# hasindu2008/slow5tools

Hardware: AMD Instinct MI355X
Metric: blow5_encode_raw_signal_throughput (higher is better)
Workload: dtype int16->u8

## Files before the change

### slow5tools_amd/csrc/deflate2_dev.h

```cpp
#pragma once

namespace s5 {

__device__ __forceinline__ uint32_t alignbit(uint32_t hi, uint32_t lo, uint32_t sh) { return __builtin_amdgcn_alignbit(hi, lo, sh); }
__device__ __forceinline__ uint32_t zbytes(uint32_t x) {
    const uint32_t t = (x & 0x7F7F7F7Fu) + 0x7F7F7F7Fu;
    return ~(t | x | 0x7F7F7F7Fu);
}
__device__ __forceinline__ uint32_t frame_mask(int a0, int first, int len) {
    const int lo = min(4, max(0, first - a0)), hi = min(4, max(0, len - a0));
    const uint32_t mh = hi >= 4 ? 0xFFFFFFFFu : (1u << (8 * hi)) - 1u;
    const uint32_t ml = lo >= 4 ? 0xFFFFFFFFu : (1u << (8 * lo)) - 1u;
    return mh & ~ml & 0x80808080u;
}
__device__ __forceinline__ int top_slot(uint32_t m) { return (31 - __clz((int)m)) >> 3; }

__device__ __forceinline__ void length_symbol(int L, uint32_t &sym, uint32_t &eb, uint32_t &ev) {
    const int l = L - 3;
    eb = 0; ev = 0;
    if (L == 258) sym = 285;
    else if (l < 8) sym = 257 + l;
    else {
        const int nb = 29 - __clz(l);
        sym = 261 + 4 * nb + ((l >> nb) & 3);
// ... 176 lines not shown
                    return C & ((Cp1 & (E | Cm1)) | (Ep & Cm1));
                };
                if (__ballot((member_of(E0, EpA) | member_of(E1, E0)) != 0u) == 0ull) {
                    carryE = (uint32_t)__builtin_amdgcn_readlane((int)E1, 63);
                    const uint32_t bA = alignbit(w0, wp, 16), bB = alignbit(w1, w0, 16);
                    atomicAdd(&wf[bA & 255u], 1u);
                    atomicAdd(&wf[(bA >> 8) & 255u], 1u);
                    atomicAdd(&wf[(bA >> 16) & 255u], 1u);
                    atomicAdd(&wf[bA >> 24], 1u);
                    atomicAdd(&wf[bB & 255u], 1u);
                    atomicAdd(&wf[(bB >> 8) & 255u], 1u);
                    atomicAdd(&wf[(bB >> 16) & 255u], 1u);
                    atomicAdd(&wf[bB >> 24], 1u);
                    const uint32_t wA = (uint32_t)(len - (256 * k + 8 * lane - 2));
                    const uint32_t sA = __builtin_amdgcn_udot4(bA, 0x01010101u, 0u, false), sB = __builtin_amdgcn_udot4(bB, 0x01010101u, 0u, false);
                    a_acc += sA + sB;
                    b_acc = __umul24(wA, sA) + __umul24(wA - 4u, sB) + b_acc;
                    d_acc = __builtin_amdgcn_udot4(bA, 0x03020100u, d_acc, false);
                    d_acc = __builtin_amdgcn_udot4(bB, 0x03020100u, d_acc, false);
                    wc.ok = false;
                    k++;
                    continue;
                }
            }
#endif
            const bool full = k > 0 && 256 * k + 256 <= len;
            const uint32_t wgt = (uint32_t)(len - (256 * k + 4 * lane - 2));
            SlabCls c;
            if (full) c = classify_slab<false>(buf32, k, len, carryE);
            else c = classify_slab<true>(buf32, k, len, carryE);
            const bool anymem = __ballot(c.member != 0u) != 0ull;
            if (full && !anymem) {
                atomicAdd(&wf[c.bytes & 255u], 1u);
                atomicAdd(&wf[(c.bytes >> 8) & 255u], 1u);
                atomicAdd(&wf[(c.bytes >> 16) & 255u], 1u);
                atomicAdd(&wf[c.bytes >> 24], 1u);
                const uint32_t s4 = __builtin_amdgcn_udot4(c.bytes, 0x01010101u, 0u, false);
                a_acc += s4;
                b_acc = __umul24(wgt, s4) + b_acc;
                d_acc = __builtin_amdgcn_udot4(c.bytes, 0x03020100u, d_acc, false);
                wc.ok = false;
                continue;
            }
            {
                uint32_t bytes = c.bytes;
                if (!full) { const uint32_t vb = c.V >> 7; bytes &= (vb << 8) - vb; }
                const uint32_t s4 = __builtin_amdgcn_udot4(bytes, 0x01010101u, 0u, false);
                a_acc += s4;
                b_acc = __umul24(wgt, s4) + b_acc;
                d_acc = __builtin_amdgcn_udot4(bytes, 0x03020100u, d_acc, false);
            }
            const uint32_t lit = c.V & ~c.member;
            if (!anymem) {
#pragma unroll
                for (int q = 0; q < 4; q++)
                    if (lit & (0x80u << (8 * q))) atomicAdd(&wf[(c.bytes >> (8 * q)) & 255u], 1u);
                if (lane == k - k0) segs = SEG_MASK;
                wc.ok = false;
                continue;
            }
            const SlabTail t = slab_tail(buf, k, c, wc);
            uint32_t tsym = 0, teb = 0, tev = 0;
            if (t.ql < 4 && t.rem >= 3) length_symbol((int)t.rem, tsym, teb, tev);
            const uint32_t ntail = t.ql < 4 ? t.nfull + (t.rem >= 3 ? 1u : t.rem) : 0u;
            const uint32_t i1 = (lit >> 7) & 1u, i2 = i1 + ((lit >> 15) & 1u), i3 = i2 + ((lit >> 23) & 1u);
            const uint32_t cnt = i3 + (lit >> 31) + ntail;
            const uint32_t incl = wave_incl_add(cnt);
            const uint32_t total = (uint32_t)__builtin_amdgcn_readlane((int)incl, 63);
            uint32_t st = 0;
            if (lane == 0) {
                st = atomicAdd(&S.lalloc, total);
                if (st < DEFL2_LIST_CAP && st + total > DEFL2_LIST_CAP) {
                    atomicMax(&S.lalloc, (uint32_t)DEFL2_LIST_CAP);
                    st = atomicAdd(&S.lalloc, total);
                }
            }
            st = (uint32_t)__builtin_amdgcn_readfirstlane((int)st);
            const bool listed = st + total <= list_cap && st + total < 65536u;
            uint16_t *tl = st < DEFL2_LIST_CAP ? tla : tlb_top - (st - DEFL2_LIST_CAP) - total - st;
            const uint32_t base = st + incl - cnt;
            const uint32_t idx[4] = {0u, i1, i2, i3};
#pragma unroll
            for (int q = 0; q < 4; q++)
                if (lit & (0x80u << (8 * q))) {
                    const uint32_t b = (c.bytes >> (8 * q)) & 255u;
                    atomicAdd(&wf[b], 1u);
                    if (listed) tl[base + idx[q] + ((uint32_t)q > t.ql ? ntail : 0u)] = (uint16_t)b;
                }
            if (t.ql < 4) {
                uint32_t at = base + (t.ql == 3 ? (lit >> 7) & 1u : 0u);
                if (t.nfull) {
                    atomicAdd(&wf[285], t.nfull);
                    nmatch += t.nfull;
                    if (listed) for (uint32_t i = 0; i < t.nfull; i++) tl[at++] = (uint16_t)285;
                }
                if (t.rem >= 3) {
                    atomicAdd(&wf[tsym], 1u);
                    nmatch += 1;
                    nextra += teb;
                    if (listed) tl[at] = (uint16_t)(tsym | (tev << 9));
                } else if (t.rem) {
                    atomicAdd(&wf[t.runbyte], t.rem);
                    if (listed) for (uint32_t i = 0; i < t.rem; i++) tl[at++] = (uint16_t)t.runbyte;
                }
            }
            if (lane == k - k0) segs = listed ? st | (total << 16) : SEG_REDO;
        }
        const uint32_t a_w = wave_sum(a_acc);
        const uint32_t b_w = wave_sum((b_acc - d_acc) % 65521u);
        const uint32_t mx = wave_sum(nmatch | (nextra << 16));
        if (lane == 0) {
            S.wad[wv] = a_w;
            S.wad[8 + wv] = b_w;
            S.wtot[16 + wv] = mx >> 16;
            S.wtot[24 + wv] = mx & 0xFFFFu;
        }
    }
    __syncthreads();
    if (dbg == 2) { z.bitpos += wfa[tid] + S.wad[tid & 15]; return; }

    const uint32_t la = S.lalloc;
    const uint32_t listb_words = poolb_ok && la > DEFL2_LIST_CAP ? (((la < list_cap ? la : list_cap) - DEFL2_LIST_CAP + 7u) >> 3) << 2 : 0u;
    const bool poolb_used = listb_words != 0u;
    if (wv == 0) {
#ifndef S5_DEFL2_ABSORB
#define S5_DEFL2_ABSORB 2
#endif
        const bool ok = assign_lengths_wave<15, NWV, true, S5_DEFL2_ABSORB>(wfa, NLIT, S.lens, S.blcount, S.bins);
        if (lane == 0) S.dbg = ok ? 0u : 1u;
    } else {
        typedef uint32_t u4a __attribute__((ext_vector_type(4)));
        u4a *o16 = reinterpret_cast<u4a *>(obuf);
        const uint32_t zend = (wf_at - listb_words) / 4;
        for (uint32_t i = (uint32_t)(wv * 64 + lane) - 64u; i < zend; i += TN - 64) o16[i] = u4a{0u, 0u, 0u, 0u};
    }
    __syncthreads();
    if (dbg == 3) { z.bitpos += S.lens[tid]; return; }
    if (tid == 0) {
        if (FUSED) put_bits(obuf, z, 64, 0x9c78u, 16);
        else obuf[0] = z.carry;
    }
    if (wv == 0) {
        if (lane == 0) {
            S.lens[DOFF] = 1; S.lens[DOFF + 1] = 1;
            S.code[DOFF] = 0u | (1u << 16); S.code[DOFF + 1] = 1u | (1u << 16);
        }
        cl_header_wave(S, 2);
    } else if (wv == 1) {
        assign_codes_wave(S.blcount, S.lens, NLIT, S.code);
    } else {
        for (int h = wv - 2; h < NWV; h += NWV - 2) {
            const uint32_t *fh = wfa + h * 288;
            const uint32_t f0 = fh[lane], f1 = fh[64 + lane], f2 = fh[128 + lane], f3 = fh[192 + lane], f4 = lane < NLIT - 256 ? fh[256 + lane] : 0u;
            uint32_t dynb = f0 * S.lens[lane] + f1 * S.lens[64 + lane] + f2 * S.lens[128 + lane] + f3 * S.lens[192 + lane] + f4 * S.lens[256 + lane];
            uint32_t fixb = 8u * (f0 + f1 + f2 + f3 + f4) + (lane >= 16 ? f2 : 0u) + f3 - (lane < 24 ? f4 : 0u);
            dynb = wave_sum(dynb);
            fixb = wave_sum(fixb);
            if (lane == 0) { S.wtot[h] = dynb; S.wtot[8 + h] = fixb; }
            uint32_t *fz = wfa + h * 288;
            fz[lane] = 0u; fz[64 + lane] = 0u; fz[128 + lane] = 0u; fz[192 + lane] = 0u;
            if (lane < NLIT - 256) fz[256 + lane] = 0u;
        }
    }
    __syncthreads();
    if (dbg == 4 || dbg == 41) { z.bitpos += S.wtot[tid & 31] + S.red[6] + S.code[tid]; return; }
    uint32_t my_dyn = 0, my_fix = 0, my_x = 0, my_m = 0;
    if (lane < NWV) { my_dyn = S.wtot[lane]; my_fix = S.wtot[8 + lane]; my_x = S.wtot[16 + lane]; my_m = S.wtot[24 + lane]; }
    auto row8_incl = [](uint32_t v) {
        v += dpp_u32<DPP_ROW_SHR1>(0, v);
        v += dpp_u32<DPP_ROW_SHR2>(0, v);
        if (NWV > 4) v += dpp_u32<DPP_ROW_SHR4>(0, v);
        return v;
    };
    const uint32_t dyn_body_all = (uint32_t)__builtin_amdgcn_readlane((int)row8_incl(my_dyn + my_x + my_m), NWV - 1);
    const uint32_t fix_body_all = (uint32_t)__builtin_amdgcn_readlane((int)row8_incl(my_fix + my_x + 5u * my_m), NWV - 1);
    const uint32_t eob_dyn = S.lens[256];
    const uint32_t hdr_dyn = 17 + 3 * S.hclen + S.red[6];
    const uint32_t dyn_total = hdr_dyn + dyn_body_all + eob_dyn;
    const uint32_t fix_total = 3 + fix_body_all + 7;
    const uint32_t sto_total = 3 + ((0u - (z.bitpos + 3)) & 7) + 32 + 8u * (uint32_t)len;
    if (!FUSED) {
        uint32_t a = 0, b = 0;
#pragma unroll
        for (int w = 0; w < NWV; w++) { a += S.wad[w]; b += S.wad[8 + w]; }
        const uint32_t nb = (uint32_t)(((uint64_t)adB + (uint64_t)len * adA + b) % 65521u);
        adA = (adA + a) % 65521u;
        adB = nb;
    }
    if (sto_total <= dyn_total && sto_total <= fix_total) {
        const uint32_t bytepos = (z.bitpos + 3 + 7) >> 3;
        publish_size(es, (bytepos + 4 + (uint32_t)len) * 8);
        uint8_t *ob8 = reinterpret_cast<uint8_t *>(obuf) + (bytepos - z.flushed * 4);
        if (poolb_used) {
            typedef uint32_t u4a __attribute__((ext_vector_type(4)));
            u4a *l16 = reinterpret_cast<u4a *>(obuf + (wf_at - listb_words));
            for (uint32_t i = tid; i < listb_words / 4; i += TN) l16[i] = u4a{0u, 0u, 0u, 0u};
        }
        __syncthreads();
        if (tid == 0) {
            put_bits(obuf, z, z.bitpos, final ? 1u : 0u, 3);
            put_bits(obuf, z, bytepos * 8, (uint32_t)len | ((~(uint32_t)len) << 16), 32);
        }
        __syncthreads();
        for (int i = tid; i < len; i += TN) ob8[4 + i] = buf[i];
        z.bitpos = (bytepos + 4 + (uint32_t)len) * 8;
        __syncthreads();
        return;
    }
    const bool use_fixed = fix_total < dyn_total || S.dbg != 0;
    const uint32_t dist_bits = use_fixed ? 5u : 1u;
    const uint32_t pos0 = z.bitpos + (use_fixed ? 3u : hdr_dyn);
    const uint32_t my_t = (use_fixed ? my_fix : my_dyn) + my_x + my_m * dist_bits;
    const uint32_t t_incl = row8_incl(my_t);
    const uint32_t total_bits = (uint32_t)__builtin_amdgcn_readlane((int)t_incl, NWV - 1);
    uint32_t wbase = pos0 + (wv ? (uint32_t)__builtin_amdgcn_readlane((int)t_incl, wv - 1) : 0u);
    const uint32_t eob = use_fixed ? fixed_code(256) : S.code[256];
    publish_size(es, pos0 + total_bits + (eob >> 16));
    if (use_fixed) {
        __syncthreads();
        for (int s = tid; s < 288; s += TN) { S.code[s] = fixed_code(s); S.lens[s] = (uint8_t)fixed_len(s); }
    }
    const bool list_ok = !poolb_used || ((pos0 + total_bits + 15u + 31u) >> 5) - z.flushed + 4u <= wf_at - listb_words;
    if (!list_ok) {
        typedef uint32_t u4a __attribute__((ext_vector_type(4)));
        u4a *l16 = reinterpret_cast<u4a *>(obuf + (wf_at - listb_words));
        for (uint32_t i = tid; i < listb_words / 4; i += TN) l16[i] = u4a{0u, 0u, 0u, 0u};
    }
    if (use_fixed || !list_ok) __syncthreads();
    if (wv == 0) {
        if (use_fixed) {
            if (lane == 0) put_bits(obuf, z, z.bitpos, (final ? 1u : 0u) | (1u << 1), 3);
        } else {
            const uint32_t hclen = S.hclen;
            if (lane == 0) put_bits(obuf, z, z.bitpos, (final ? 1u : 0u) | (2u << 1) | ((S.hlit - 257) << 3) | (1u << 8) | ((hclen - 4) << 13), 17);
            if (lane < (int)hclen) {
                const int order[19] = {16, 17, 18, 0, 8, 7, 9, 6, 10, 5, 11, 4, 12, 3, 13, 2, 14, 1, 15};
                put_bits(obuf, z, z.bitpos + 17 + 3 * lane, S.cllens[order[lane]], 3);
            }
            const int ncl = S.ncl;
            uint32_t cv[5], cn[5], sum = 0;
#pragma unroll
            for (int q = 0; q < 5; q++) {
                const int e = 5 * lane + q;
                cv[q] = 0; cn[q] = 0;
                if (e < ncl) {
                    const uint32_t ent = S.clseq[e];
                    const uint32_t sym = ent & 31, cc = S.clcode[sym], cl = cc >> 16;
                    const uint32_t eb = sym == 16 ? 2 : sym == 17 ? 3 : sym == 18 ? 7 : 0;
                    cv[q] = (cc & 0xFFFF) | ((ent >> 5) << cl);
                    cn[q] = cl + eb;
                }
                sum += cn[q];
            }
            uint32_t p = z.bitpos + 17 + 3 * hclen + wave_incl_add(sum) - sum;
#pragma unroll
            for (int q = 0; q < 5; q++) {
                if (cn[q]) put_bits(obuf, z, p, cv[q], cn[q]);
                p += cn[q];
            }
        }
    }
    if (dbg == 5) { z.bitpos += wbase; return; }

    {
        auto or_bits = [&](uint32_t pos, uint64_t v, uint32_t nb) {
            const uint32_t w = (pos >> 5) - z.flushed, sh = pos & 31;
            const uint64_t lo = v << sh;
            atomicOr(&obuf[w], (uint32_t)lo);
            atomicOr(&obuf[w + 1], (uint32_t)(lo >> 32));
            if (sh + nb > 64) atomicOr(&obuf[w + 2], (uint32_t)(v >> (64 - sh)));
        };
        auto lit4 = [&](uint32_t bytes, uint64_t &v, uint32_t &nb) {
            const uint32_t c0 = S.code[bytes & 255u], c1 = S.code[(bytes >> 8) & 255u], c2 = S.code[(bytes >> 16) & 255u], c3 = S.code[bytes >> 24];
            const uint32_t n0 = c0 >> 16, n1 = c1 >> 16, n2 = c2 >> 16, n3 = c3 >> 16;
            const uint32_t lo = (c0 & 0xFFFFu) | ((c1 & 0xFFFFu) << n0), nlo = n0 + n1;
            const uint32_t hi = (c2 & 0xFFFFu) | ((c3 & 0xFFFFu) << n2), nhi = n2 + n3;
            v = (uint64_t)lo | ((uint64_t)hi << nlo);
            nb = nlo + nhi;
        };
        for (int k = k0; k < k1; k++) {
            const uint32_t seg = (uint32_t)__builtin_amdgcn_readlane((int)segs, k - k0);
            if (seg == SEG_FAST && k + 1 < k1 && (uint32_t)__builtin_amdgcn_readlane((int)segs, k + 1 - k0) == SEG_FAST) {
                const int d0 = 64 * k + 2 * lane;
                const uint32_t wp = buf32[d0 - 1], w0 = buf32[d0], w1 = buf32[d0 + 1];
                uint64_t vA, vB;
                uint32_t nA, nB;
                lit4(alignbit(w0, wp, 16), vA, nA);
                lit4(alignbit(w1, w0, 16), vB, nB);
                const uint32_t nb = nA + nB;
                const uint32_t incl = wave_incl_add(nb);
                const uint32_t pos = wbase + incl - nb;
                or_bits(pos, vA, nA);
                or_bits(pos + nA, vB, nB);
                wbase += (uint32_t)__builtin_amdgcn_readlane((int)incl, 63);
                k++;
                continue;
            }
            if (seg == SEG_FAST) {
                const int di = 64 * k + lane;
                uint64_t v;
                uint32_t nb;
                lit4(alignbit(buf32[di], buf32[di - 1], 16), v, nb);
                const uint32_t incl = wave_incl_add(nb);
                or_bits(wbase + incl - nb, v, nb);
                wbase += (uint32_t)__builtin_amdgcn_readlane((int)incl, 63);
                continue;
            }
// ... 111 lines not shown
```

### slow5tools_amd/csrc/deflate_dev.h

```cpp
#pragma once
#include "dev_common.h"

namespace s5 {

constexpr int DEFL_BLK = NT * 64;
constexpr int NLIT = 286;
constexpr int DOFF = 288;

template <int CAP>
struct BuildScratchT {
    alignas(16) uint32_t lf[CAP];
    alignas(16) uint32_t nf[CAP];
    uint16_t npar[CAP];
    uint16_t rsym[CAP];
};
struct SortScratch {
    uint32_t bm[64 * 9];
    uint32_t cnt[64];
    uint32_t ovl[288];
};
struct BuildScratch : BuildScratchT<288> { SortScratch sort; };

struct DeflShared {
    alignas(16) uint32_t freq[320];
// ... 242 lines not shown
            l[q] = lq;
            csum += 1u << (MAXL - lq);
            c[q] = lq > 1 ? 1u << (MAXL - lq) : HUGE_C;
            b[q] = min(63u, (uint32_t)((float)(f[q] << ls) * inv) >> (ls - lq));
        } else { l[q] = 0; c[q] = HUGE_C; b[q] = 0; }
    }
    const uint32_t used_c = wave_sum(csum);
    if (used_c > (1u << MAXL)) return false;
    uint32_t R = (1u << MAXL) - used_c;
    int guard = 0;
    while (R) {
        if (ABSORB > 0 && guard == ABSORB) {
            uint32_t nun = 0;
#pragma unroll
            for (int q = 0; q < 5; q++) nun += (5 * lane + q < n && f[q] == 0u) ? 1u : 0u;
            const uint32_t incl = wave_incl_add(nun);
            if ((uint32_t)__builtin_amdgcn_readlane((int)incl, 63) >= (uint32_t)__popc(R)) {
                uint32_t r = R;
                const uint32_t skip = incl - nun;
#pragma unroll
                for (uint32_t i = 0; i < (uint32_t)MAXL; i++) if (i < skip) r &= r - 1u;
#pragma unroll
                for (int q = 0; q < 5; q++)
                    if (5 * lane + q < n && f[q] == 0u && r) {
                        l[q] = MAXL - (__ffs((int)r) - 1);
                        r &= r - 1u;
                    }
                R = 0;
                break;
            }
        }
        if (++guard > 40) return false;
        bins[lane] = 0;
        wave_sync();
#pragma unroll
        for (int q = 0; q < 5; q++)
            if (c[q] <= R) atomicAdd(&bins[b[q]], c[q]);
        wave_sync();
        const uint32_t hr = bins[63 - lane];
        const uint32_t incl = wave_incl_add(hr);
        const uint64_t fit = __ballot(incl <= R);
        const int nfit = ~fit ? __ffsll((long long)~fit) - 1 : 64;
        const uint32_t whole = nfit ? (uint32_t)__builtin_amdgcn_readlane((int)incl, nfit - 1) : 0u;
        const uint64_t below = nfit < 64 ? (__ballot(hr != 0u) >> nfit) << nfit : 0ull;
        const uint32_t thr = 64u - (uint32_t)nfit;
        const uint32_t pb = below ? 63u - (uint32_t)(__ffsll((long long)below) - 1) : 0xFFFFu;
        const uint32_t Rold = R;
        R -= whole;
        uint32_t mine = 0;
#pragma unroll
        for (int q = 0; q < 5; q++) mine += (c[q] <= Rold && b[q] == pb) ? c[q] : 0u;
        uint32_t run = wave_incl_add(mine) - mine, got = 0;
#pragma unroll
        for (int q = 0; q < 5; q++) {
            bool sel = c[q] <= Rold && b[q] >= thr && b[q] != pb;
            if (c[q] <= Rold && b[q] == pb) { run += c[q]; if (run <= R) { sel = true; got += c[q]; } }
            if (sel) {
                l[q] -= 1;
                c[q] = l[q] > 1 ? c[q] << 1 : HUGE_C;
                b[q] >>= 1;
            }
        }
        R -= wave_sum(got);
    }
#pragma unroll
    for (int q = 0; q < 5; q++) {
        const int s = 5 * lane + q;
        if (s < n) {
            lens[s] = (uint8_t)l[q];
            if (l[q]) atomicAdd(&blcount[l[q]], 1u);
        }
    }
    wave_sync();
    return true;
}

__device__ __forceinline__ void assign_codes_wave(const uint32_t *blcount, const uint8_t *lens, int n, uint32_t *code_out) {
    {
        uint32_t next[16];
        uint32_t c = 0;
        next[0] = 0;
#pragma unroll
        for (int b = 1; b < 16; b++) {
            c = (c + (b > 1 ? (uint32_t)__builtin_amdgcn_readfirstlane((int)blcount[b - 1]) : 0u)) << 1;
            next[b] = c;
        }
        for (int base = 0; base < n; base += 64) {
            const int s = base + lane_id();
            const int l = s < n ? lens[s] : 0;
            uint32_t mine = 0;
#pragma unroll
            for (int b = 1; b < 16; b++) {
                const uint64_t mask = __ballot(l == b);
                if (mask == 0) continue;
                const uint32_t below = __builtin_amdgcn_mbcnt_hi((uint32_t)(mask >> 32), __builtin_amdgcn_mbcnt_lo((uint32_t)mask, 0u));
                if (l == b) mine = next[b] + below;
                next[b] += __popcll(mask);
            }
            if (s < n) code_out[s] = l ? ((__brev(mine) >> (32 - l)) | ((uint32_t)l << 16)) : 0u;
        }
    }
    wave_sync();
}

__device__ __forceinline__ int fixed_len(int s) { return s < 144 ? 8 : s < 256 ? 9 : s < 280 ? 7 : 8; }
__device__ __forceinline__ uint32_t fixed_code(int s) {
    uint32_t c, l;
    if (s < 144) { c = 0x30 + s; l = 8; }
    else if (s < 256) { c = 0x190 + (s - 144); l = 9; }
    else if (s < 280) { c = s - 256; l = 7; }
    else { c = 0xC0 + (s - 280); l = 8; }
    return (__brev(c) >> (32 - l)) | (l << 16);
}

__device__ __forceinline__ void cl_header_wave(DeflShared &S, int hdist) {
    const int lane = lane_id();
    if (lane < 20) S.clfreq[lane] = 0;
    int hl = lane < 29 && S.lens[257 + lane] ? 258 + lane : 257;
    const int hlit = __builtin_amdgcn_readlane(wave_incl_max(hl), 63), n = hlit + hdist;
    if (lane == 0) S.hlit = (uint32_t)hlit;
    wave_sync();
    {
        constexpr int PP = 5;
        const int p0 = PP * lane;
        int v[PP];
        int prevv = -1;
        if (p0 - 1 >= 0 && p0 - 1 < n) prevv = p0 - 1 < hlit ? S.lens[p0 - 1] : S.lens[DOFF + p0 - 1 - hlit];
        uint32_t bk = 0;
#pragma unroll
        for (int q = 0; q < PP; q++) {
            const int p = p0 + q;
            v[q] = p < n ? (p < hlit ? S.lens[p] : S.lens[DOFF + p - hlit]) : -2 - q;
            if (p < n && v[q] != (q == 0 ? prevv : v[q - 1])) bk |= 1u << q;
        }
        const int local_last = bk ? p0 + 31 - __clz(bk) : -1;
        const int local_first = bk ? p0 + __ffs(bk) - 1 : n;
        int lastb = wave_incl_max(local_last);
        lastb = __shfl_up(lastb, 1);
        if (lane == 0) lastb = -1;
        int nextb = wave_suffix_incl_min(local_first);
        nextb = __shfl_down(nextb, 1);
        if (lane == 63) nextb = n;
        uint32_t ent[PP], nent = 0;
#pragma unroll
        for (int q = 0; q < PP; q++) {
            const int p = p0 + q;
            ent[q] = 0xFFFFFFFFu;
            if (p >= n) continue;
            const uint32_t lo = bk & ((2u << q) - 1), hi = bk >> (q + 1);
            const int s = lo ? p0 + 31 - __clz(lo) : lastb;
            const int e = hi ? p + __ffs(hi) : nextb;
            const int R = e - s, rel = p - s;
            if (v[q] == 0) {
                const int c = rel / 138, off = rel - c * 138, Lc = min(138, R - c * 138);
                if (Lc >= 11) { if (off == 0) ent[q] = 18u | ((uint32_t)(Lc - 11) << 5); }
                else if (Lc >= 3) { if (off == 0) ent[q] = 17u | ((uint32_t)(Lc - 3) << 5); }
                else ent[q] = 0;
            } else if (rel == 0) {
                ent[q] = (uint32_t)v[q];
            } else {
                const int mm = rel - 1, c = mm / 6, off = mm - c * 6, Lc = min(6, R - 1 - c * 6);
                if (Lc >= 3) { if (off == 0) ent[q] = 16u | ((uint32_t)(Lc - 3) << 5); }
                else ent[q] = (uint32_t)v[q];
            }
            nent += ent[q] != 0xFFFFFFFFu;
        }
        const uint32_t incl = wave_incl_add(nent);
        uint32_t at = incl - nent;
#pragma unroll
        for (int q = 0; q < PP; q++)
            if (ent[q] != 0xFFFFFFFFu) {
                S.clseq[at++] = (uint16_t)ent[q];
                atomicAdd(&S.clfreq[ent[q] & 31], 1u);
            }
        if (lane == 63) S.ncl = incl;
    }
    wave_sync();
    {
        static constexpr uint32_t CLA[19] = {0x30001, 0x7002f, 0x7006f, 0x7001f, 0x7005f, 0x50003, 0x50013, 0x5000b, 0x5001b, 0x50007,
                                             0x30005, 0x20000, 0x20002, 0x7003f, 0x00000, 0x00000, 0x50017, 0x6000f, 0x7007f};
        static constexpr uint32_t CLB[19] = {0x30002, 0x60017, 0x7002f, 0x7006f, 0x60037, 0x5000b, 0x40005, 0x5001b, 0x50007, 0x4000d,
                                             0x30006, 0x30001, 0x20000, 0x7001f, 0x7005f, 0x7003f, 0x40003, 0x6000f, 0x7007f};
        const uint32_t ca = lane < 19 ? CLA[lane] : 0u, cb = lane < 19 ? CLB[lane] : 0u;
        const uint32_t f = lane < 19 ? S.clfreq[lane] : 0u;
        const uint32_t eb = lane == 16 ? 2u : lane == 17 ? 3u : lane == 18 ? 7u : 0u;
        const uint32_t costA = wave_sum(f * ((ca >> 16) + eb) + ((f && !(ca >> 16)) ? (1u << 24) : 0u));
        const uint32_t costB = wave_sum(f * ((cb >> 16) + eb));
        const bool useA = costA <= costB;
        if (lane < 19) { const uint32_t c = useA ? ca : cb; S.clcode[lane] = c; S.cllens[lane] = (uint8_t)(c >> 16); }
        if (lane == 0) { S.red[6] = useA ? costA : costB; S.hclen = useA ? 18u : 19u; }
    }
}

template <int TN = NT>
__device__ __forceinline__ void flush_words(uint32_t *obuf, uint32_t *out32, ZOut &z, bool final_all, uint32_t n_words = 0xFFFFFFFFu) {
    const int tid = threadIdx.x;
    const uint32_t full = final_all ? (z.bitpos + 31) >> 5 : z.bitpos >> 5;
    const uint32_t n = n_words != 0xFFFFFFFFu ? n_words : full - z.flushed;
    {
        typedef uint32_t u4u __attribute__((ext_vector_type(4), aligned(4)));
        typedef uint32_t u4a __attribute__((ext_vector_type(4)));
        const u4a *s16 = reinterpret_cast<const u4a *>(obuf);
        const uint32_t nv = n >> 2;
        for (uint32_t j = tid; j < nv; j += TN) {
            const uint32_t w = z.flushed + 4u * j;
            const u4a v = s16[j];
            if (w >= 2) *reinterpret_cast<u4u *>(out32 + w) = v;
            else { out32[w + 2] = v.z; out32[w + 3] = v.w; }
        }
        for (uint32_t i = 4u * nv + tid; i < n; i += TN) {
            const uint32_t w = z.flushed + i;
            if (w >= 2) out32[w] = obuf[i];
        }
    }
    if (final_all) return;
    __syncthreads();
    const uint32_t partial = obuf[n];
    __syncthreads();
    for (uint32_t i = tid; i <= n; i += TN) obuf[i] = i == 0 ? partial : 0u;
    __syncthreads();
    z.flushed = full;
}

}
#include "deflate2_dev.h"
namespace s5 {

template <typename M>
__device__ __forceinline__ uint32_t zlib_frame_fused(DeflShared &S, uint32_t *obuf, uint32_t obuf_words, const uint8_t *pay,
                                                     uint32_t plen, ZOut &z, uint32_t dbg = 0, EarlySize es = EarlySize{nullptr, 0}, uint32_t gen_hint = 0,
                                                     bool prepared = false) {
    const int tid = threadIdx.x;
    z.bitpos = 80;
    z.flushed = 0;
    uint32_t adA = 1, adB = 0;
    deflate_block2<1, NT>(S, obuf, obuf_words, pay, (int)plen, true, z, adA, adB, dbg, es, gen_hint, prepared);
    if (dbg) return 16;
    z.bitpos = (z.bitpos + 7) & ~7u;
    if (tid == 0 && plen) {
        uint32_t a = 0, b = 0;
        for (int w = 0; w < NW; w++) { a += S.wad[w]; b += S.wad[8 + w]; }
        adB = (uint32_t)(((uint64_t)plen + b) % 65521u);
        adA = (1u + a) % 65521u;
    }
    if (tid == 0) put_bits(obuf, z, z.bitpos, __builtin_bswap32((adB << 16) | adA), 32);
    z.bitpos += 32;
    __syncthreads();
    return z.bitpos >> 3;
}

template <typename M>
__device__ __forceinline__ uint32_t zlib_compress_fused(DeflShared &S, uint32_t *obuf, uint32_t obuf_words,
                                                        const uint8_t *pay, uint32_t plen, uint8_t *out, uint32_t dbg = 0, uint32_t gen_hint = 0, bool prepared = false) {
    ZOut z;
    const uint32_t total = zlib_frame_fused<M>(S, obuf, obuf_words, pay, plen, z, dbg, EarlySize{nullptr, 0}, gen_hint, prepared);
    if (dbg) {
        if (threadIdx.x == 0) *reinterpret_cast<uint32_t *>(out) = z.bitpos;
        if (dbg == 41 && threadIdx.x < 20) reinterpret_cast<uint32_t *>(out)[4 + threadIdx.x] = threadIdx.x < 19 ? S.clfreq[threadIdx.x] : S.red[6];
        return 16;
    }
    flush_words(obuf, reinterpret_cast<uint32_t *>(out), z, true);
    if (threadIdx.x == 0) *reinterpret_cast<uint64_t *>(out) = (uint64_t)(total - 8);
    return total;
}

constexpr uint64_t LB_MASK = (1ull << 62) - 1;
__device__ __forceinline__ uint64_t wave_sum64(uint64_t v) {
#pragma unroll
    for (int d = 32; d >= 1; d >>= 1) v += __shfl_xor(v, d);
    return v;
}
template <int E = 1>
__device__ __forceinline__ uint64_t lookback_offset(unsigned long long *st, uint32_t r, uint64_t mysize, uint32_t *err, bool published) {
    const int lane = lane_id();
    if (!published && lane == 0) __hip_atomic_store(&st[r], (1ull << 62) | mysize, __ATOMIC_RELAXED, __HIP_MEMORY_SCOPE_AGENT);
    uint64_t acc = 0;
    long long base = (long long)r - 1;
    uint32_t spins = 0;
    for (;;) {
        uint64_t v[E];
#pragma unroll
        for (int e = 0; e < E; e++) {
            const long long idx = base - 64 * e - lane;
            v[e] = idx >= 0 ? __hip_atomic_load(&st[idx], __ATOMIC_RELAXED, __HIP_MEMORY_SCOPE_AGENT) : (2ull << 62);
        }
        int outcome = 0;
#pragma unroll
        for (int e = 0; e < E; e++) {
            if (outcome) continue;
            const uint32_t f = (uint32_t)(v[e] >> 62);
            const uint64_t m0 = __ballot(f == 0), m2 = __ballot(f == 2);
            const int first0 = m0 ? __ffsll((long long)m0) - 1 : 64;
            const int first2 = m2 ? __ffsll((long long)m2) - 1 : 64;
            if (first2 < first0) {
                acc += lane <= first2 ? (v[e] & LB_MASK) : 0ull;
                outcome = 1;
            } else {
                acc += lane < first0 ? (v[e] & LB_MASK) : 0ull;
                if (first0 < 64) { base -= 64 * e + first0; outcome = 2; }
            }
        }
        if (outcome == 1) break;
        if (outcome == 0) { base -= 64 * E; continue; }
        if (++spins > (1u << 22)) { if (lane == 0) *err = 1; break; }
        __builtin_amdgcn_s_sleep(2);
    }
    const uint64_t excl = wave_sum64(acc);
    if (lane == 0) __hip_atomic_store(&st[r], (2ull << 62) | (excl + mysize), __ATOMIC_RELAXED, __HIP_MEMORY_SCOPE_AGENT);
    return excl;
}
__device__ __forceinline__ void copy_record_out(const uint32_t *obuf, uint32_t total, uint8_t *dst) {
    const int tid = threadIdx.x;
    typedef uint32_t u4u __attribute__((ext_vector_type(4), aligned(1)));
    typedef uint32_t u4a __attribute__((ext_vector_type(4)));
// ... 10 lines not shown
```

### slow5tools_amd/csrc/kernels.hip

```cpp
#include <hip/hip_runtime.h>
#include <limits.h>
#include <stdint.h>
#include <stdio.h>
#include <stdlib.h>
#include <string.h>

#include <atomic>
#include <mutex>
#include <type_traits>
#include <vector>

#include "../../include/slow5gpu.h"
#include "deflate_dev.h"
#include "lz_dev.h"
#include "inflate_dev.h"
#include "inflate_simt_dev.h"
#include "inflate_par_dev.h"
#include "zstd_dev.h"
#include "zstd_enc_dev.h"
#include "svb_dev.h"
#include "exzd_dev.h"
#include "order_dev.h"
#include "enc_plan.h"

using namespace s5;

extern "C" void s5gpu_set_error(const char *fmt, ...);
int s5host_set_option(const char *key, long value);
extern uint32_t s5host_generation;
static_assert(s5plan::BLK == (uint32_t)DEFL_BLK && s5plan::SIG_SVB_ZD == S5GPU_SIG_SVB_ZD && s5plan::SIG_EX_ZD == S5GPU_SIG_EX_ZD, "enc_plan.h restates these");

#define HIP_TRY(x)                                                                                   \
    do {                                                                                             \
        hipError_t e_ = (x);                                                                         \
        if (e_ != hipSuccess) {                                                                      \
            s5gpu_set_error("%s failed: %s (%s:%d)", #x, hipGetErrorString(e_), __FILE__, __LINE__); \
            return S5GPU_ERR_HIP;                                                                    \
        }                                                                                            \
    } while (0)

extern __shared__ __attribute__((aligned(16))) uint8_t smem[];

constexpr uint32_t S_BYTES = (sizeof(DeflShared) + 15u) & ~15u;
constexpr uint32_t BZ_BYTES = (sizeof(BuildScratch) + 15u) & ~15u;
constexpr uint32_t B_BYTES = NW * 288u * 4u + 64u;
constexpr uint32_t OVF = 0xFFFFFFFFu;

struct EncParams {
    s5gpu_encode_args_t a;
    uint32_t obuf_words;
    uint32_t pay_cap;
    uint32_t dbg;
    uint32_t zseq;
    uint32_t tier = 0;
};

static uint32_t g_fused_tier2 = 0;
static uint32_t g_zstd_sequences = 1;

__device__ __forceinline__ uint32_t payload_bound_dev(const s5gpu_read_desc_t &d, int sig_method) {
    const uint32_t n = d.n_samples;
    const uint32_t sig = sig_method == S5GPU_SIG_SVB_ZD ? 4 + ((n + 3) >> 2) + 3 * n
                       : sig_method == S5GPU_SIG_EX_ZD ? 24 + 2 * (((n + 3) >> 2) + 4 * n) + n : 2 * n;
    return d.hdr_len + 8 + sig + d.aux_len;
}

template <bool EXZD = false>
__device__ __forceinline__ uint32_t build_payload(const s5gpu_encode_args_t &a, const s5gpu_read_desc_t &d,
                                                  uint8_t *pay, uint32_t cap, uint32_t *ws, uint32_t *red = nullptr) {
    const int tid = threadIdx.x;
    const uint32_t n = d.n_samples;
    if constexpr (EXZD) {
        const uint32_t fixed_x = d.hdr_len + 8 + d.aux_len;
        if (fixed_x + 16 > cap) return OVF;
        const uint8_t *hdr = a.hdr + d.hdr_off;
        for (uint32_t i = tid; i < d.hdr_len; i += NT) pay[i] = hdr[i];
        uint8_t *lenp = pay + d.hdr_len;
        const uint32_t blen = exzd_encode_wg(a.sig + d.sig_off, n, lenp + 8, ws, red, cap - fixed_x);
        if (blen == EXZD_ERR) return OVF;
        if (tid < 8) lenp[tid] = tid < 4 ? (uint8_t)(blen >> (8 * tid)) : 0;
        if (d.aux_len) {
            const uint8_t *aux = a.aux + d.aux_off;
            uint8_t *ap = lenp + 8 + blen;
            for (uint32_t i = tid; i < d.aux_len; i += NT) ap[i] = aux[i];
        }
        return d.hdr_len + 8 + blen + d.aux_len;
    } else {
    const bool svb = a.sig_method == S5GPU_SIG_SVB_ZD;
    const uint32_t nk = (n + 3) >> 2;
    const uint32_t fixed = d.hdr_len + 8 + (svb ? 4 + nk : 0) + d.aux_len;
    if (fixed > cap || (svb ? n : 2 * n) > cap - fixed) return OVF;
    const uint8_t *hdr = a.hdr + d.hdr_off;
    for (uint32_t i = tid; i < d.hdr_len; i += NT) pay[i] = hdr[i];
    uint8_t *lenp = pay + d.hdr_len;
    uint8_t *sigp = lenp + 8;
    const int16_t *sig = a.sig + d.sig_off;
    uint64_t L;
    uint32_t sig_bytes;
    if (svb) {
        uint8_t *keys = sigp + 4;
        uint8_t *data = keys + nk;
        uint32_t total = 0;
        const uint32_t room = cap - fixed;
        for (uint32_t t0 = 0; t0 < n; t0 += SVB_TILE) {
            const uint32_t t = svb_encode_tile(sig, n, t0, keys + (t0 >> 2), data + total, ws, room - total, true);
            if (t > room - total) return OVF;
            total += t;
        }
        L = 4ull + nk + total;
        sig_bytes = (uint32_t)L;
        if (tid < 4) sigp[tid] = (uint8_t)(n >> (8 * tid));
    } else {
        L = n;
        sig_bytes = 2 * n;
        const uint8_t *src = reinterpret_cast<const uint8_t *>(sig);
        for (uint32_t i = tid; i < sig_bytes; i += NT) sigp[i] = src[i];
    }
    if (tid < 8) lenp[tid] = (uint8_t)(L >> (8 * tid));
    if (d.aux_len) {
        const uint8_t *aux = a.aux + d.aux_off;
        uint8_t *ap = sigp + sig_bytes;
        for (uint32_t i = tid; i < d.aux_len; i += NT) ap[i] = aux[i];
    }
    return d.hdr_len + 8 + sig_bytes + d.aux_len;
    }
}

__device__ __forceinline__ uint32_t build_payload_hbm(const s5gpu_encode_args_t &a, const s5gpu_read_desc_t &d, uint8_t *pay,
                                                      uint32_t *ws, uint32_t *tile_keys, uint32_t *tile_data) {
    const int tid = threadIdx.x;
    const uint32_t n = d.n_samples;
    if (a.sig_method == S5GPU_SIG_EX_ZD) return build_payload<true>(a, d, pay, OVF - 1, ws, tile_keys );
    if (a.sig_method != S5GPU_SIG_SVB_ZD) return build_payload(a, d, pay, OVF - 1, ws);
    const uint32_t nk = (n + 3) >> 2;
    const uint8_t *hdr = a.hdr + d.hdr_off;
    for (uint32_t i = tid; i < d.hdr_len; i += NT) pay[i] = hdr[i];
    uint8_t *lenp = pay + d.hdr_len;
    uint8_t *sigp = lenp + 8;
    const int16_t *sig = a.sig + d.sig_off;
    uint8_t *keys = sigp + 4;
    uint8_t *data = keys + nk;
    uint32_t total = 0;
    for (uint32_t t0 = 0; t0 < n; t0 += SVB_TILE) {
        const uint32_t t = svb_encode_tile(sig, n, t0, reinterpret_cast<uint8_t *>(tile_keys), reinterpret_cast<uint8_t *>(tile_data), ws, OVF - 1);
        __syncthreads();
        const uint32_t tk = (min(n - t0, (uint32_t)SVB_TILE) + 3) >> 2;
        copy_record_out(tile_keys, tk, keys + (t0 >> 2));
        copy_record_out(tile_data, t, data + total);
        total += t;
        __syncthreads();
    }
    const uint64_t L = 4ull + nk + total;
    if (tid < 4) sigp[tid] = (uint8_t)(n >> (8 * tid));
    if (tid < 8) lenp[tid] = (uint8_t)(L >> (8 * tid));
    if (d.aux_len) {
        const uint8_t *aux = a.aux + d.aux_off;
        uint8_t *ap = sigp + (uint32_t)L;
        for (uint32_t i = tid; i < d.aux_len; i += NT) ap[i] = aux[i];
    }
    return d.hdr_len + 8 + (uint32_t)L + d.aux_len;
}

__device__ __forceinline__ uint32_t run_heavy_front(const s5gpu_encode_args_t &a, const s5gpu_read_desc_t &d) {
    return a.sig_method == S5GPU_SIG_SVB_ZD ? d.hdr_len + 12u + ((d.n_samples + 3u) >> 2) : 0u;
}

#ifndef S5_FUSED_HINT
#define S5_FUSED_HINT(a, d) run_heavy_front(a, d)
#endif

#ifndef S5_FUSED_WG_PER_CU
#define S5_FUSED_WG_PER_CU 8
#endif
template <typename M, bool EXZD = false, int WPS = S5_FUSED_WG_PER_CU>
__global__ __launch_bounds__(NT, WPS) void k_encode_fused(EncParams p) {
    const uint32_t r = blockIdx.x;
    if (p.tier == 2 && p.a.out_len[r] != 0) return;
    DeflShared &S = *reinterpret_cast<DeflShared *>(smem);
    uint32_t *obuf = reinterpret_cast<uint32_t *>(smem + S_BYTES);
    uint8_t *pay = smem + S_BYTES + 4u * p.obuf_words;
    const s5gpu_read_desc_t d = p.a.desc[r];
    deflate2_prepare<NT>(S, obuf, p.obuf_words);
    const uint32_t plen = build_payload<EXZD>(p.a, d, pay, p.pay_cap, S.ws, S.red);
    if (plen == OVF) {
        if (threadIdx.x == 0 && p.tier != 1) {
            const uint32_t at = atomicAdd(&p.a.ovf[0], 1u);
            p.a.ovf[1 + at] = r;
        }
        return;
    }
    __syncthreads();
    if (p.dbg == 1) {
        if (threadIdx.x == 0) p.a.out_len[r] = plen + pay[plen - 1];
        return;
    }
    uint8_t *out = p.a.slots + d.out_off;
    const uint32_t total = zlib_compress_fused<M>(S, obuf, p.obuf_words, pay, plen, out, p.dbg, S5_FUSED_HINT(p.a, d), true);
    if (threadIdx.x == 0) p.a.out_len[r] = total;
}

#ifndef S5_LB_E
#define S5_LB_E 1
#endif
struct StreamParams {
    unsigned long long *state;
    uint32_t *ctl;
    uint8_t *stream;
    uint64_t *rec_off;
};
template <typename M, bool EXZD = false>
__global__ __launch_bounds__(NT, S5_FUSED_WG_PER_CU) void k_encode_stream(EncParams p, StreamParams sp) {
    __shared__ uint32_t s_r;
    __shared__ uint64_t s_off;
    DeflShared &S = *reinterpret_cast<DeflShared *>(smem);
    uint32_t *obuf = reinterpret_cast<uint32_t *>(smem + S_BYTES);
    uint8_t *pay = smem + S_BYTES + 4u * p.obuf_words;
#ifdef S5_ES_NOTICKET
    const uint32_t r = blockIdx.x;
#else
    if (threadIdx.x == 0) s_r = atomicAdd(&sp.ctl[1], 1u);
    __syncthreads();
    const uint32_t r = s_r;
#endif
    const s5gpu_read_desc_t d = p.a.desc[r];
    deflate2_prepare<NT>(S, obuf, p.obuf_words);
    const uint32_t plen = build_payload<EXZD>(p.a, d, pay, p.pay_cap, S.ws, S.red);
    uint32_t total = 0;
    if (plen == OVF) {
        if (threadIdx.x == 0) atomicAdd(&sp.ctl[0], 1u);
    } else {
        __syncthreads();
        ZOut z;
        total = zlib_frame_fused<M>(S, obuf, p.obuf_words, pay, plen, z, 0, EarlySize{sp.state, r}, S5_FUSED_HINT(p.a, d), true);
        if (threadIdx.x == 0) { obuf[0] = total - 8; obuf[1] = 0; }
    }
    if (wave_id() == 0) {
        const uint64_t off = lookback_offset<S5_LB_E>(sp.state, r, total, &sp.ctl[2], plen != OVF);
        if (lane_id() == 0) {
            s_off = off;
            sp.rec_off[r] = off;
            if (r == p.a.n_reads - 1) sp.rec_off[p.a.n_reads] = off + total;
            p.a.out_len[r] = total;
        }
    }
    __syncthreads();
    if (total) copy_record_out(obuf, total, sp.stream + s_off);
}

__device__ __forceinline__ uint32_t park_offset(const s5gpu_read_desc_t &d, int sig_method) {
    return (d.slot_cap - payload_bound_dev(d, sig_method)) & ~15u;
}

#ifndef S5_PACK_WG
#define S5_PACK_WG 8
#endif
__global__ __launch_bounds__(NT, S5_PACK_WG) void k_pack(EncParams p, int mode, const uint32_t *ord) {
    __shared__ uint32_t ws[16];
    __shared__ __attribute__((aligned(16))) uint32_t tile_keys[SVB_TILE / 16 + 4];
// ... 1865 lines not shown
```

### slow5tools_amd/csrc/svb_dev.h

```cpp
#pragma once
#include "dev_common.h"

namespace s5 {

constexpr int SVB_TILE = NT * 16;

struct SvbTileLane {
    uint32_t z[16];
    uint32_t key, nbytes;
    int valid;
};
#ifndef S5_SVB_PACKED
#define S5_SVB_PACKED 1
#endif
__device__ __forceinline__ void svb_tile_classify(const int16_t *__restrict__ sig, uint32_t n, uint32_t t0, SvbTileLane &T) {
    const int tid = threadIdx.x;
    const uint32_t i0 = t0 + 16u * tid;
    const int valid = i0 >= n ? 0 : (int)min(16u, n - i0);
#if S5_SVB_PACKED
    {
        typedef unsigned short us2 __attribute__((ext_vector_type(2)));
        typedef short ss2 __attribute__((ext_vector_type(2)));
        auto U = [](uint32_t v) { return __builtin_bit_cast(us2, v); };
        auto W = [](us2 v) { return __builtin_bit_cast(uint32_t, v); };
        uint32_t w[8] = {0u, 0u, 0u, 0u, 0u, 0u, 0u, 0u}, pw = 0u;
        bool ok = valid == 0;
        if (valid == 16) {
            const uint4 a = *reinterpret_cast<const uint4 *>(sig + i0);
            const uint4 b = *reinterpret_cast<const uint4 *>(sig + i0 + 8);
            w[0] = a.x; w[1] = a.y; w[2] = a.z; w[3] = a.w; w[4] = b.x; w[5] = b.y; w[6] = b.z; w[7] = b.w;
            if (i0 > 0) pw = *reinterpret_cast<const uint32_t *>(sig + i0 - 2);
            uint32_t rng = W(U(pw) + us2{0x4000, 0x4000});
#pragma unroll
            for (int j = 0; j < 8; j++) rng |= W(U(w[j]) + us2{0x4000, 0x4000});
            ok = (rng & 0x80008000u) == 0u;
        }
        if (__ballot(!ok) == 0ull) {
            uint32_t A = 0, B = 0;
#pragma unroll
            for (int j = 0; j < 8; j++) {
                const uint32_t xp = __builtin_amdgcn_alignbit(w[j], j ? w[j - 1] : pw, 16);
                const ss2 d = __builtin_bit_cast(ss2, w[j]) - __builtin_bit_cast(ss2, xp);
                const us2 z = __builtin_bit_cast(us2, d) << us2{1, 1} ^ __builtin_bit_cast(us2, d >> ss2{15, 15});
                const us2 c = __builtin_elementwise_min(z >> us2{8, 8}, us2{1, 1});
                T.z[2 * j] = (uint32_t)z.x;
                T.z[2 * j + 1] = (uint32_t)z.y;
                if (j < 4) A |= W(c) << (4 * j); else B |= W(c) << (4 * (j - 4));
            }
            const uint32_t key = ((A | (A >> 14)) & 0xFFFFu) | ((B | (B >> 14)) << 16);
            T.key = key;
            T.nbytes = valid == 16 ? 16u + (uint32_t)__popc(key) : 0u;
            T.valid = valid;
            return;
        }
    }
#endif
    int x[16];
    int prev = 0;
    if (valid == 16) {
        const int4 a = *reinterpret_cast<const int4 *>(sig + i0);
        const int4 b = *reinterpret_cast<const int4 *>(sig + i0 + 8);
        const int w[8] = {a.x, a.y, a.z, a.w, b.x, b.y, b.z, b.w};
#pragma unroll
        for (int q = 0; q < 8; q++) {
            x[2 * q] = (int)(short)(w[q] & 0xFFFF);
            x[2 * q + 1] = w[q] >> 16;
        }
    } else {
#pragma unroll
        for (int q = 0; q < 16; q++) x[q] = q < valid ? (int)sig[i0 + q] : 0;
    }
    if (valid > 0 && i0 > 0) prev = sig[i0 - 1];
    uint32_t key = 0, nbytes = 0;
    const bool full = valid == 16;
#pragma unroll
    for (int q = 0; q < 16; q++) {
        const int d = x[q] - prev;
        prev = x[q];
        T.z[q] = ((uint32_t)d << 1) ^ (uint32_t)(d >> 31);
    }
    if (full) {
#pragma unroll
        for (int q = 0; q < 16; q++) {
            const uint32_t code = (T.z[q] > 0xFFu ? 1u : 0u) + (T.z[q] >> 16);
            key |= code << (2 * q);
            nbytes += code;
        }
        nbytes += 16;
    } else {
#pragma unroll
        for (int q = 0; q < 16; q++) {
            const uint32_t code = (T.z[q] > 0xFFu) + (T.z[q] > 0xFFFFu);
            if (q < valid) {
                key |= code << (2 * q);
                nbytes += code + 1;
            }
        }
    }
    T.key = key;
    T.nbytes = nbytes;
    T.valid = valid;
}
__device__ __forceinline__ void svb_tile_write(const SvbTileLane &T, uint8_t *keys, uint8_t *dp) {
    const int tid = threadIdx.x;
    if (T.valid == 16) {
#pragma unroll
        for (int q = 0; q < 16; q++) {
            *dp++ = (uint8_t)T.z[q];
            if (T.z[q] > 0xFFu) {
                *dp++ = (uint8_t)(T.z[q] >> 8);
                if (T.z[q] > 0xFFFFu) *dp++ = (uint8_t)(T.z[q] >> 16);
            }
        }
    } else {
#pragma unroll
        for (int q = 0; q < 16; q++) {
            if (q < T.valid) {
                *dp++ = (uint8_t)T.z[q];
                if (T.z[q] > 0xFFu) *dp++ = (uint8_t)(T.z[q] >> 8);
                if (T.z[q] > 0xFFFFu) *dp++ = (uint8_t)(T.z[q] >> 16);
            }
        }
    }
    const int nk = (T.valid + 3) >> 2;
#pragma unroll
    for (int q = 0; q < 4; q++)
        if (q < nk) keys[4 * tid + q] = (uint8_t)(T.key >> (8 * q));
}
__device__ __forceinline__ uint32_t svb_encode_tile(const int16_t *__restrict__ sig, uint32_t n, uint32_t t0,
                                                    uint8_t *keys, uint8_t *data, uint32_t *ws, uint32_t room, bool ws_fresh = false) {
    SvbTileLane T;
    svb_tile_classify(sig, n, t0, T);
    if (t0 == 0 && !ws_fresh) __syncthreads();
    uint32_t total;
    const uint32_t off = block_excl_add_alt(T.nbytes, ws, total, t0 / (uint32_t)SVB_TILE);
    if (total > room) return total;
    svb_tile_write(T, keys, data + off);
    return total;
}

__device__ __forceinline__ uint32_t svb_key_bytes(uint32_t n) { return (uint32_t)(((uint64_t)n + 3u) >> 2); }
__device__ __forceinline__ bool svb_count_fits(uint32_t n, uint64_t L) { return 4ull + svb_key_bytes(n) + n <= L; }

constexpr uint32_t SVB_STAGE = 4u * SVB_TILE + 16u;
__device__ __forceinline__ uint32_t svb_decode_tile(const uint8_t *keys, const uint8_t *data, const uint8_t *data_end,
                                                    uint32_t n, uint32_t t0, int16_t *__restrict__ out, int &carry,
                                                    int &err, uint32_t *ws, uint8_t *stage) {
    const int tid = threadIdx.x;
    const uint32_t i0 = t0 + 16u * tid;
    const int valid = i0 >= n ? 0 : (int)min(16u, n - i0);
    const int nk = (valid + 3) >> 2;
    uint32_t key = 0;
#pragma unroll
    for (int q = 0; q < 4; q++)
        if (q < nk) key |= (uint32_t)keys[4 * tid + q] << (8 * q);
    uint32_t nbytes = 0;
#pragma unroll
    for (int q = 0; q < 16; q++)
        if (q < valid) nbytes += ((key >> (2 * q)) & 3) + 1;
    uint32_t total;
    const uint32_t off = block_excl_add(nbytes, ws, total);
    {
        const uint32_t have = data < data_end ? (uint32_t)min((uint64_t)total, (uint64_t)(data_end - data)) : 0u;
        typedef uint32_t v4u __attribute__((ext_vector_type(4), aligned(1)));
        typedef uint32_t v4a __attribute__((ext_vector_type(4)));
        for (uint32_t k = 16u * tid; k < have; k += 16u * NT) {
            if (k + 16 <= have) *reinterpret_cast<v4a *>(stage + k) = *reinterpret_cast<const v4u *>(data + k);
            else for (uint32_t j = k; j < have; j++) stage[j] = data[j];
        }
        __syncthreads();
    }
    const uint8_t *dp = stage + off;
    const bool ok = !(valid > 0 && data + off + nbytes > data_end);
    if (!ok) { err = 1; }
    int d[16];
    int sum = 0;
#pragma unroll
    for (int q = 0; q < 16; q++) {
        d[q] = 0;
        if (q < valid && ok) {
            const uint32_t code = (key >> (2 * q)) & 3;
            uint32_t zz = dp[0];
            if (code > 0) zz |= (uint32_t)dp[1] << 8;
            if (code > 1) zz |= (uint32_t)dp[2] << 16;
            if (code > 2) zz |= (uint32_t)dp[3] << 24;
            dp += code + 1;
            d[q] = (int)(zz >> 1) ^ -(int)(zz & 1);
        }
        sum += d[q];
    }
    uint32_t tsum;
    const uint32_t before = block_excl_add((uint32_t)sum, ws, tsum);
    int acc = carry + (int)before;
    if (valid == 16) {
        uint32_t w[8];
#pragma unroll
        for (int q = 0; q < 8; q++) {
            acc += d[2 * q];
            const uint32_t lo = (uint32_t)acc & 0xFFFFu;
            acc += d[2 * q + 1];
            w[q] = lo | ((uint32_t)acc << 16);
        }
        uint4 *o = reinterpret_cast<uint4 *>(out + i0);
        o[0] = make_uint4(w[0], w[1], w[2], w[3]);
        o[1] = make_uint4(w[4], w[5], w[6], w[7]);
    } else {
#pragma unroll
        for (int q = 0; q < 16; q++)
            if (q < valid) { acc += d[q]; out[i0 + q] = (int16_t)acc; }
    }
    carry += (int)tsum;
    return total;
}

constexpr uint32_t SVB_WTILE = 64u * 16u;
constexpr uint32_t SVB_WSTAGE = 4u * SVB_WTILE + 16u;
template <bool STAGED = true>
__device__ __forceinline__ uint32_t svb_decode_tile_wave(const uint8_t *keys, const uint8_t *data, const uint8_t *data_end, uint32_t n, uint32_t t0,
                                                         int16_t *__restrict__ out, int &carry, int &err, uint8_t *stage) {
    const int lane = lane_id();
    const uint32_t i0 = t0 + 16u * (uint32_t)lane;
    const int valid = i0 >= n ? 0 : (int)min(16u, n - i0);
    const int nk = (valid + 3) >> 2;
    uint32_t key = 0;
    if (valid == 16) {
        typedef uint32_t u1 __attribute__((aligned(1)));
        key = *reinterpret_cast<const u1 *>(keys + 4 * lane);
    } else {
#pragma unroll
        for (int q = 0; q < 4; q++)
            if (q < nk) key |= (uint32_t)keys[4 * lane + q] << (8 * q);
    }
    uint32_t nbytes;
    {
        const uint32_t km = valid >= 16 ? key : key & ((1u << (2 * valid)) - 1u);
        uint32_t c = (km & 0x33333333u) + ((km >> 2) & 0x33333333u);
        c = (c + (c >> 4)) & 0x0F0F0F0Fu;
        nbytes = (uint32_t)valid + ((c * 0x01010101u) >> 24);
    }
    const uint32_t incl = wave_incl_add(nbytes);
    const uint32_t off = incl - nbytes;
    const uint32_t total = (uint32_t)__builtin_amdgcn_readlane((int)incl, 63);
    if (STAGED) {
        const uint32_t have = data < data_end ? (uint32_t)min((uint64_t)total, (uint64_t)(data_end - data)) : 0u;
        typedef uint32_t v4u __attribute__((ext_vector_type(4), aligned(1)));
        typedef uint32_t v4a __attribute__((ext_vector_type(4)));
        for (uint32_t k = 16u * (uint32_t)lane; k < have; k += 16u * 64u) {
            if (k + 16 <= have) *reinterpret_cast<v4a *>(stage + k) = *reinterpret_cast<const v4u *>(data + k);
            else for (uint32_t j = k; j < have; j++) stage[j] = data[j];
        }
        wave_sync();
    }
    const uint8_t *dp = (STAGED ? stage : data) + off;
    const bool ok = !(valid > 0 && data + off + nbytes > data_end);
    if (!ok) err = 1;
    int dlt[16];
    int sum = 0;
#pragma unroll
    for (int q = 0; q < 16; q++) {
        dlt[q] = 0;
        if (q < valid && ok) {
            const uint32_t code = (key >> (2 * q)) & 3;
            uint32_t zz = dp[0];
            if (code > 0) zz |= (uint32_t)dp[1] << 8;
            if (code > 1) zz |= (uint32_t)dp[2] << 16;
            if (code > 2) zz |= (uint32_t)dp[3] << 24;
            dp += code + 1;
            dlt[q] = (int)(zz >> 1) ^ -(int)(zz & 1);
        }
        sum += dlt[q];
    }
    const uint32_t incl2 = wave_incl_add((uint32_t)sum);
    int acc = carry + (int)(incl2 - (uint32_t)sum);
    if (valid == 16) {
        uint32_t w[8];
#pragma unroll
        for (int q = 0; q < 8; q++) {
            acc += dlt[2 * q];
            const uint32_t lo = (uint32_t)acc & 0xFFFFu;
            acc += dlt[2 * q + 1];
            w[q] = lo | ((uint32_t)acc << 16);
        }
        uint4 *o = reinterpret_cast<uint4 *>(out + i0);
        o[0] = make_uint4(w[0], w[1], w[2], w[3]);
        o[1] = make_uint4(w[4], w[5], w[6], w[7]);
    } else {
#pragma unroll
        for (int q = 0; q < 16; q++)
            if (q < valid) { acc += dlt[q]; out[i0 + q] = (int16_t)acc; }
    }
// ... 7 lines not shown
```

Before: 687.1.

## Pack SVB zigzag values as 16-bit pairs and write bytes with carry-chained cursors

```diff
diff --git a/slow5tools_amd/csrc/deflate2_dev.h b/slow5tools_amd/csrc/deflate2_dev.h
--- a/slow5tools_amd/csrc/deflate2_dev.h
+++ b/slow5tools_amd/csrc/deflate2_dev.h
@@ -352,7 +352,7 @@
         for (int h = wv - 2; h < NWV; h += NWV - 2) {
             const uint32_t *fh = wfa + h * 288;
             const uint32_t f0 = fh[lane], f1 = fh[64 + lane], f2 = fh[128 + lane], f3 = fh[192 + lane], f4 = lane < NLIT - 256 ? fh[256 + lane] : 0u;
-            uint32_t dynb = f0 * S.lens[lane] + f1 * S.lens[64 + lane] + f2 * S.lens[128 + lane] + f3 * S.lens[192 + lane] + f4 * S.lens[256 + lane];
+            uint32_t dynb = __umul24(f0, S.lens[lane]) + __umul24(f1, S.lens[64 + lane]) + __umul24(f2, S.lens[128 + lane]) + __umul24(f3, S.lens[192 + lane]) + __umul24(f4, S.lens[256 + lane]);
             uint32_t fixb = 8u * (f0 + f1 + f2 + f3 + f4) + (lane >= 16 ? f2 : 0u) + f3 - (lane < 24 ? f4 : 0u);
             dynb = wave_sum(dynb);
             fixb = wave_sum(fixb);
diff --git a/slow5tools_amd/csrc/deflate_dev.h b/slow5tools_amd/csrc/deflate_dev.h
--- a/slow5tools_amd/csrc/deflate_dev.h
+++ b/slow5tools_amd/csrc/deflate_dev.h
@@ -418,14 +418,14 @@
             const int e = hi ? p + __ffs(hi) : nextb;
             const int R = e - s, rel = p - s;
             if (v[q] == 0) {
-                const int c = rel / 138, off = rel - c * 138, Lc = min(138, R - c * 138);
+                const int c = (rel >= 138) + (rel >= 276), off = rel - c * 138, Lc = min(138, R - c * 138);
                 if (Lc >= 11) { if (off == 0) ent[q] = 18u | ((uint32_t)(Lc - 11) << 5); }
                 else if (Lc >= 3) { if (off == 0) ent[q] = 17u | ((uint32_t)(Lc - 3) << 5); }
                 else ent[q] = 0;
             } else if (rel == 0) {
                 ent[q] = (uint32_t)v[q];
             } else {
-                const int mm = rel - 1, c = mm / 6, off = mm - c * 6, Lc = min(6, R - 1 - c * 6);
+                const int mm = rel - 1, c = (int)(__umul24((uint32_t)mm, 171u) >> 10), off = mm - c * 6, Lc = min(6, R - 1 - c * 6);
                 if (Lc >= 3) { if (off == 0) ent[q] = 16u | ((uint32_t)(Lc - 3) << 5); }
                 else ent[q] = (uint32_t)v[q];
             }
diff --git a/slow5tools_amd/csrc/kernels.hip b/slow5tools_amd/csrc/kernels.hip
--- a/slow5tools_amd/csrc/kernels.hip
+++ b/slow5tools_amd/csrc/kernels.hip
@@ -103,7 +103,7 @@
         uint32_t total = 0;
         const uint32_t room = cap - fixed;
         for (uint32_t t0 = 0; t0 < n; t0 += SVB_TILE) {
-            const uint32_t t = svb_encode_tile(sig, n, t0, keys + (t0 >> 2), data + total, ws, room - total, true);
+            const uint32_t t = svb_encode_tile<true>(sig, n, t0, keys + (t0 >> 2), data + total, ws, room - total, true);
             if (t > room - total) return OVF;
             total += t;
         }
diff --git a/slow5tools_amd/csrc/svb_dev.h b/slow5tools_amd/csrc/svb_dev.h
--- a/slow5tools_amd/csrc/svb_dev.h
+++ b/slow5tools_amd/csrc/svb_dev.h
@@ -9,10 +9,17 @@
     uint32_t z[16];
     uint32_t key, nbytes;
     int valid;
+    bool pairs;
 };
 #ifndef S5_SVB_PACKED
 #define S5_SVB_PACKED 1
 #endif
+__device__ __forceinline__ uint32_t svb_pair_codes(uint32_t z) {
+    uint32_t c;
+    asm("v_pk_lshrrev_b16 %0, 8, %1 op_sel_hi:[0,1]\n\tv_pk_min_u16 %0, %0, 1 op_sel_hi:[1,0]" : "=v"(c) : "v"(z));
+    return c;
+}
+template <bool PAIRS = false>
 __device__ __forceinline__ void svb_tile_classify(const int16_t *__restrict__ sig, uint32_t n, uint32_t t0, SvbTileLane &T) {
     const int tid = threadIdx.x;
     const uint32_t i0 = t0 + 16u * tid;
@@ -42,15 +49,22 @@
                 const uint32_t xp = __builtin_amdgcn_alignbit(w[j], j ? w[j - 1] : pw, 16);
                 const ss2 d = __builtin_bit_cast(ss2, w[j]) - __builtin_bit_cast(ss2, xp);
                 const us2 z = __builtin_bit_cast(us2, d) << us2{1, 1} ^ __builtin_bit_cast(us2, d >> ss2{15, 15});
-                const us2 c = __builtin_elementwise_min(z >> us2{8, 8}, us2{1, 1});
-                T.z[2 * j] = (uint32_t)z.x;
-                T.z[2 * j + 1] = (uint32_t)z.y;
-                if (j < 4) A |= W(c) << (4 * j); else B |= W(c) << (4 * (j - 4));
+                uint32_t c;
+                if constexpr (PAIRS) {
+                    c = svb_pair_codes(W(z));
+                    T.z[j] = W(z);
+                } else {
+                    c = W(__builtin_elementwise_min(z >> us2{8, 8}, us2{1, 1}));
+                    T.z[2 * j] = (uint32_t)z.x;
+                    T.z[2 * j + 1] = (uint32_t)z.y;
+                }
+                if (j < 4) A |= c << (4 * j); else B |= c << (4 * (j - 4));
             }
             const uint32_t key = ((A | (A >> 14)) & 0xFFFFu) | ((B | (B >> 14)) << 16);
             T.key = key;
             T.nbytes = valid == 16 ? 16u + (uint32_t)__popc(key) : 0u;
             T.valid = valid;
+            T.pairs = PAIRS;
             return;
         }
     }
@@ -100,9 +114,77 @@
     T.key = key;
     T.nbytes = nbytes;
     T.valid = valid;
-}
+    T.pairs = false;
+}
+typedef __attribute__((address_space(3))) uint8_t svb_lds_u8;
+struct SvbCursorLds {
+    uint32_t a;
+    __device__ __forceinline__ svb_lds_u8 *at() const { return (svb_lds_u8 *)(uintptr_t)a; }
+};
+struct SvbCursorHbm {
+    uint8_t *base;
+    uint32_t a;
+    __device__ __forceinline__ uint8_t *at() const { return base + a; }
+};
+__device__ __forceinline__ void svb_pair_step(uint32_t cur, uint32_t z, uint32_t &n0, uint32_t &n1, uint64_t &two0, uint64_t &two1) {
+    asm("v_cmp_lt_u16_e64 %2, %5, %6\n\t"
+        "v_cmp_lt_u32_e64 %3, %7, %6\n\t"
+        "s_nop 0\n\t"
+        "v_addc_co_u32_e64 %0, vcc, 0, %4, %2\n\t"
+        "v_addc_co_u32_e64 %1, vcc, 0, %0, %3"
+        : "=&v"(n0), "=&v"(n1), "=&s"(two0), "=&s"(two1)
+        : "v"(cur), "s"(0xFFu), "v"(z), "s"(0xFFFFFFu)
+        : "vcc");
+}
+__device__ __forceinline__ void svb_write_key4(uint8_t *kp, uint32_t key) {
+    uint32_t ks = key >> 8, one = 1u;
+    asm("" : "+v"(ks));
+    asm("" : "+s"(one));
+    uint8_t *kq = kp + one;
+    kp[0] = (uint8_t)key;
+    kq[0] = (uint8_t)ks;
+    kp[2] = (uint8_t)(key >> 16);
+    kq[2] = (uint8_t)(ks >> 16);
+}
+template <class Cursor>
+__device__ __forceinline__ void svb_tile_write_packed(const SvbTileLane &T, uint8_t *keys, Cursor c) {
+    if (T.valid == 0) return;
+#pragma unroll
+    for (int j = 0; j < 8; j++) {
+        const uint32_t z = T.z[j];
+        uint32_t s = z >> 8;
+        asm("" : "+v"(s));
+        uint32_t n0, n1;
+        uint64_t two0, two1;
+        svb_pair_step(c.a, z, n0, n1, two0, two1);
+        c.at()[2 * j] = (uint8_t)z;
+        if (__builtin_amdgcn_inverse_ballot_w64(two0)) c.at()[2 * j + 1] = (uint8_t)s;
+        c.a = n0;
+        c.at()[2 * j + 1] = (uint8_t)(z >> 16);
+        if (__builtin_amdgcn_inverse_ballot_w64(two1)) c.at()[2 * j + 2] = (uint8_t)(s >> 16);
+        c.a = n1;
+    }
+    svb_write_key4(keys + 4 * threadIdx.x, T.key);
+}
+__device__ __forceinline__ bool svb_in_lds(const uint8_t *p) {
+#if defined(__HIP_DEVICE_COMPILE__)
+    return __builtin_amdgcn_is_shared(p);
+#else
+    (void)p;
+    return false;
+#endif
+}
+template <bool PAIRS = false>
 __device__ __forceinline__ void svb_tile_write(const SvbTileLane &T, uint8_t *keys, uint8_t *dp) {
     const int tid = threadIdx.x;
+    if constexpr (PAIRS) {
+        if (T.pairs) {
+            if (svb_in_lds(dp)) svb_tile_write_packed(T, keys, SvbCursorLds{(uint32_t)(uintptr_t)(svb_lds_u8 *)dp});
+            else svb_tile_write_packed(T, keys, SvbCursorHbm{dp, 0u});
+            return;
+        }
+        if (T.valid == 0) return;
+    }
     if (T.valid == 16) {
 #pragma unroll
         for (int q = 0; q < 16; q++) {
@@ -112,6 +194,7 @@
                 if (T.z[q] > 0xFFFFu) *dp++ = (uint8_t)(T.z[q] >> 16);
             }
         }
+        if constexpr (PAIRS) { svb_write_key4(keys + 4 * tid, T.key); return; }
     } else {
 #pragma unroll
         for (int q = 0; q < 16; q++) {
@@ -127,15 +210,16 @@
     for (int q = 0; q < 4; q++)
         if (q < nk) keys[4 * tid + q] = (uint8_t)(T.key >> (8 * q));
 }
+template <bool PAIRS = false>
 __device__ __forceinline__ uint32_t svb_encode_tile(const int16_t *__restrict__ sig, uint32_t n, uint32_t t0,
                                                     uint8_t *keys, uint8_t *data, uint32_t *ws, uint32_t room, bool ws_fresh = false) {
     SvbTileLane T;
-    svb_tile_classify(sig, n, t0, T);
+    svb_tile_classify<PAIRS>(sig, n, t0, T);
     if (t0 == 0 && !ws_fresh) __syncthreads();
     uint32_t total;
     const uint32_t off = block_excl_add_alt(T.nbytes, ws, total, t0 / (uint32_t)SVB_TILE);
     if (total > room) return total;
-    svb_tile_write(T, keys, data + off);
+    svb_tile_write<PAIRS>(T, keys, data + off);
     return total;
 }
 
```

After: 686.0. No clear change (-0.2%).
